# KLab/YAIK

Measured on AMD Instinct MI355X. Metric: Mpix/s tile encode (alpha reject + 7 gradient passes + 8x8 range quant), 8K RGBA, higher is better.
Workload: dtype u8/int32 (+f32 mode-selection sums)

## Files before the change

yaik_amd/csrc/yk_encode2.hip:

```cpp
#include "yk_common.h"
#include "yk_curves.h"
#include "yk_device.h"
#include <mutex>

__constant__ float c_curve2[6][16] = YK_CURVE_TABLE;

#define LS YK_LSTRIDE
#ifdef YK_TEST_HOOKS
#define YK2_ABLATE(bit) ((P.ablate & (bit)) != 0)
#else
#define YK2_ABLATE(bit) false
#endif

__device__ __forceinline__ int y2_byte(uint32_t w, int ch) { return (w >> (8 * ch)) & 255; }
__device__ __forceinline__ uint32_t y2_absdiff(uint32_t a, uint32_t b) { uint32_t r; asm("v_sad_u32 %0, %1, %2, 0" : "=v"(r) : "v"(a), "v"(b)); return r; }
__device__ __forceinline__ int y2_round6(int v) { return (v & ~3) | (v >> 6); }
__device__ __forceinline__ int y2_round6p(int v) { v = min(v + 1, 255); return (v & ~3) | (v >> 6); }

typedef short y2s2 __attribute__((ext_vector_type(2)));
typedef unsigned short y2u2 __attribute__((ext_vector_type(2)));
__device__ __forceinline__ y2u2 y2_u2(uint32_t w) { return __builtin_bit_cast(y2u2, w); }
__device__ __forceinline__ y2s2 y2_s2(y2u2 v) { return __builtin_bit_cast(y2s2, v); }
__device__ __forceinline__ y2u2 y2_splat(int v) { const unsigned short t = (unsigned short)v; return (y2u2){ t, t }; }
__device__ __forceinline__ y2s2 y2_splats(int v) { const short t = (short)v; return (y2s2){ t, t }; }
__device__ __forceinline__ y2s2 y2_rg(uint32_t p) { return y2_s2(y2_u2(__builtin_amdgcn_perm(0u, p, 0x010C000Cu) ^ 0x80008000u)); }
__device__ __forceinline__ y2s2 y2_bb(uint32_t pEven, uint32_t pOdd) { return y2_s2(y2_u2(__builtin_amdgcn_perm(pOdd, pEven, 0x060C020Cu) ^ 0x80008000u)); }
#define YK2_LATN 85
#ifdef YK2_STATS
__device__ unsigned long long g_y2_stats[192];
#define YK2_STAT(i, n) do { if (lane == 0) atomicAdd(&g_y2_stats[(i)], (unsigned long long)(n)); } while (0)
extern "C" int yk_debug_path_stats(unsigned long long* out, int clear) {
    hipError_t e = hipMemcpyFromSymbol(out, HIP_SYMBOL(g_y2_stats), sizeof(g_y2_stats));
    if (e == hipSuccess && clear) { static unsigned long long z[192]; e = hipMemcpyToSymbol(HIP_SYMBOL(g_y2_stats), z, sizeof(z)); }
    return (int)e;
}
#else
#define YK2_STAT(i, n) do { } while (0)
#endif

__device__ __forceinline__ constexpr int y2_cell_x(int m) { return (m & 1) | ((m >> 1) & 2); }
__device__ __forceinline__ constexpr int y2_cell_y(int m) { return ((m >> 1) & 1) | ((m >> 2) & 2); }
template <int NX, int NY> __device__ __forceinline__ constexpr unsigned long long y2_origin() {
    unsigned long long m = 0;
    for (int i = 0; i < 16; i++) if ((y2_cell_x(i) % NX) == 0 && (y2_cell_y(i) % NY) == 0) m |= 1ULL << i;
    return m * 0x0001000100010001ULL;
}
template <int NX, int NY> __device__ __forceinline__ unsigned long long y2_fold(unsigned long long m) {
    if (NX >= 2) m |= m >> 1;
    if (NY >= 2) m |= m >> 2;
    if (NX == 4) m |= m >> 4;
    if (NY == 4) m |= m >> 8;
    return m;
}
template <int NX, int NY> __device__ __forceinline__ unsigned long long y2_spread(unsigned long long m) {
    if (NX >= 2) m |= m << 1;
    if (NY >= 2) m |= m << 2;
    if (NX == 4) m |= m << 4;
    if (NY == 4) m |= m << 8;
    return m;
}

__device__ __forceinline__ constexpr int y2_pass_sx(int id) { return id < 2 ? 4 : (id < 5 ? 3 : 2); }
__device__ __forceinline__ constexpr int y2_pass_sy(int id) { return id == 0 || id == 2 ? 4 : (id == 1 || id == 3 || id == 5 ? 3 : 2); }
template <int SX, int SY> __device__ __forceinline__ constexpr int y2_pass_id() {
    for (int id = 0; id < 7; id++) if (y2_pass_sx(id) == SX && y2_pass_sy(id) == SY) return id;
    return -1;
}
struct Y2Pass {
    const uint32_t* s_lat; int lat;
    int cx, cy;
    const y2s2 (&rg)[16]; const y2s2 (&bb)[8];
    unsigned long long deadLanes; bool stripInside;
    int gxCell, gyCell, w, h;
    int rf;
    uint32_t* s_bm; int bxCell, byCell;
    const uint32_t* s_pix; uint8_t* s_list; uint32_t* s_tf;
    int lane;
};
struct Y2Window { y2s2 loO, hiO, loR, hiR; };
__device__ __forceinline__ Y2Window y2_window(const int rf) {
    const int loO = -256 * rf, hiO = 256 * rf + 255;
    return { y2_splats(loO), y2_splats(hiO), y2_splats(loO - 127), y2_splats(hiO - 127) };
}
template <int SX, int SY> __device__ __forceinline__ unsigned long long y2_viable(const Y2Pass pass, const unsigned long long cov) {
    constexpr int TX = 1 << SX, TY = 1 << SY, NX = TX / 4, NY = TY / 4;
    unsigned long long viable = y2_origin<NX, NY>() & ~cov & ~y2_fold<NX, NY>(pass.deadLanes);
    if (!pass.stripInside) {
        const int tgx = pass.gxCell - (pass.cx & (NX - 1)) * 4, tgy = pass.gyCell - (pass.cy & (NY - 1)) * 4;
        viable &= __ballot((tgx + TX <= pass.w) && (tgy + TY <= pass.h));
    }
    return viable;
}
template <int SX, int SY> __device__ __forceinline__ int y2_bitmap_bit(const int bxCell, const int byCell) {
    const int tbx = bxCell >> SX, tby = byCell >> SY;
    if (SX == 4 && SY == 4) return 0 + tby * 4 + tbx;
    if (SX == 4 && SY == 3) return 32 + tby * 4 + tbx;
    if (SX == 3 && SY == 4) return 64 + tby * 8 + tbx;
    if (SX == 3 && SY == 3) return 96 + tby * 8 + tbx;
    if (SX == 3 && SY == 2) return 160 + (tby >> 3) * 64 + (tby & 7) * 8 + tbx;
    if (SX == 2 && SY == 3) return 288 + (tbx >> 3) * 64 + tby * 8 + (tbx & 7);
    return 416 + ((tby >> 3) * 2 + (tbx >> 3)) * 64 + (tby & 7) * 8 + (tbx & 7);
}

template <int SX, int SY, int SXB = SX, int SYB = SY>
__device__ __forceinline__ void y2_accept(const Y2Pass pass, unsigned long long& cov, const unsigned long long accept, const unsigned long long acceptB = 0ULL) {
    cov |= y2_spread<(1 << SX) / 4, (1 << SY) / 4>(accept) | y2_spread<(1 << SXB) / 4, (1 << SYB) / 4>(acceptB);
    if ((accept | acceptB) != 0ULL && __builtin_amdgcn_inverse_ballot_w64(accept | acceptB)) {
        int bit = y2_bitmap_bit<SX, SY>(pass.bxCell, pass.byCell);
        if ((SXB != SX || SYB != SY) && __builtin_amdgcn_inverse_ballot_w64(acceptB)) bit = y2_bitmap_bit<SXB, SYB>(pass.bxCell, pass.byCell);
        atomicOr(&pass.s_bm[bit >> 5], 1u << (bit & 31));
    }
    __builtin_amdgcn_wave_barrier();
}

template <int SX, int SY>
__device__ __forceinline__ bool y2_compact_sweep(const Y2Pass pass, const unsigned long long viable, unsigned long long& cov, unsigned long long& evaluated) {
    constexpr int NX = (1 << SX) / 4, NY = (1 << SY) / 4, kPassId = y2_pass_id<SX, SY>();
    const uint32_t* const s_lat = pass.s_lat; const uint32_t* const s_pix = pass.s_pix; uint8_t* const s_list = pass.s_list; uint32_t* const s_tf = pass.s_tf;
    const int lane = pass.lane;
    const Y2Window W = y2_window(pass.rf);
    const unsigned long long cells = y2_spread<NX, NY>(viable);
    const int nCells = __popcll(cells);
    if (nCells > 16) return false;
    YK2_STAT(kPassId * 10 + 1, 1); YK2_STAT(kPassId * 10 + 7, nCells);
    constexpr bool kHasNext = kPassId >= 3 && kPassId <= 5;
    constexpr int SXB = kHasNext ? y2_pass_sx(kPassId + 1) : SX, SYB = kHasNext ? y2_pass_sy(kPassId + 1) : SY;
    constexpr int NXB = (1 << SXB) / 4, NYB = (1 << SYB) / 4;
    unsigned long long viableB = 0ULL, cellsB = 0ULL;
    int nB = 0;
#ifndef YK2_NO_GROUP
    if (kHasNext) {
        viableB = y2_viable<SXB, SYB>(pass, cov);
        cellsB = y2_spread<NXB, NYB>(viableB);
        nB = __popcll(cellsB);
        if (nB == 0 || nCells + nB > 16) { viableB = 0ULL; cellsB = 0ULL; nB = 0; }
    }
#endif
    const int rank = (int)__builtin_amdgcn_mbcnt_hi((uint32_t)(cells >> 32), __builtin_amdgcn_mbcnt_lo((uint32_t)cells, 0u));
    const bool mine = __builtin_amdgcn_inverse_ballot_w64(cells);
    if (mine) s_list[rank] = (uint8_t)lane;
    if (kHasNext && nB != 0) {
        YK2_STAT(140 + kPassId - 3, 1); YK2_STAT(150 + kPassId - 3, nB);
        const int rankB = (int)__builtin_amdgcn_mbcnt_hi((uint32_t)(cellsB >> 32), __builtin_amdgcn_mbcnt_lo((uint32_t)cellsB, 0u));
        if (__builtin_amdgcn_inverse_ballot_w64(cellsB)) s_list[nCells + rankB] = (uint8_t)lane;
    }
    s_tf[lane] = 0u; s_tf[64 + lane] = 0u;
    __builtin_amdgcn_fence(__ATOMIC_RELEASE, "wavefront"); __builtin_amdgcn_wave_barrier(); __builtin_amdgcn_fence(__ATOMIC_ACQUIRE, "wavefront");
    const int j = lane & 15, r = lane >> 4;
    const bool act = j < nCells + nB;
    const bool isB = kHasNext && j >= nCells;
    const int c = (int)s_list[act ? j : 0];
    const int q2 = c >> 4, cy2 = y2_cell_y(c & 15), cx2 = y2_cell_x(c & 15);
    constexpr int kInTile = (NX > 1 ? 1 : 0) | (NY > 1 ? 2 : 0) | (NX > 2 ? 4 : 0) | (NY > 2 ? 8 : 0);
    constexpr int kInTileB = (NXB > 1 ? 1 : 0) | (NYB > 1 ? 2 : 0) | (NXB > 2 ? 4 : 0) | (NYB > 2 ? 8 : 0);
    const int nxL = isB ? NXB : NX, nyL = isB ? NYB : NY;
    const int shx = isB ? 4 - SXB : 4 - SX, shy = isB ? 4 - SYB : 4 - SY;
    const int dcx2 = cx2 & (nxL - 1), dcy2 = cy2 & (nyL - 1);
    const int orig = c & ~(isB ? kInTileB : kInTile);
    const int fsh = isB ? 3 : 0;
    const int lo2 = cy2 * 17 + q2 * 4 + cx2 - dcy2 * 17 - dcx2;
    const int oTR = nxL, oBL = nyL * 17;
    const y2u2 wyr = y2_splat(16 - ((dcy2 * 4 + r) << shy));
    const y2u2 lxc = y2_splat(16 - ((dcx2 * 4) << shx));
    const y2u2 shx2 = y2_splat(shx);
    const uint4 pr = *reinterpret_cast<const uint4*>(&s_pix[(cy2 * 4 + r) * LS + q2 * 16 + cx2 * 4]);
    const y2s2 rgc[4] = { y2_rg(pr.x), y2_rg(pr.y), y2_rg(pr.z), y2_rg(pr.w) }, bbc[2] = { y2_bb(pr.x, pr.y), y2_bb(pr.z, pr.w) };
    y2s2 mnc[5], mxc[5];
    auto rowC = [&](const unsigned mask) {
        y2u2 Sc[5], stc[5];
#pragma unroll
        for (int t = 0; t < 5; t++) {
            if (!((mask >> t) & 1u)) continue;
            const uint32_t* lt = s_lat + t * YK2_LATN + lo2;
            const y2u2 TL = y2_u2(lt[0]), TR = y2_u2(lt[oTR]), BL = y2_u2(lt[oBL]), BR = y2_u2(lt[oBL + oTR]);
            const y2u2 e16 = (BL - BR) << 4, g = TR - BR, f = TL - BL - g;
            const y2u2 c2 = (g << 4) + f * lxc;
            Sc[t] = ((BR << 8) + e16 * lxc + c2 * wyr) ^ y2_splat(0x8000);
            stc[t] = (e16 + f * wyr) << shx2;
        }
#pragma unroll
        for (int i = 0; i < 4; i++) {
            const y2s2 c01 = rgc[i], cb = bbc[i >> 1];
            const y2s2 cc[4] = { __builtin_shufflevector(c01, c01, 0, 0), __builtin_shufflevector(c01, c01, 1, 1),
                                 (i & 1) ? __builtin_shufflevector(cb, cb, 1, 1) : __builtin_shufflevector(cb, cb, 0, 0), c01 };
#pragma unroll
            for (int t = 0; t < 4; t++) {
                if (!((mask >> t) & 1u)) continue;
                const y2s2 D = __builtin_elementwise_sub_sat(y2_s2(Sc[t]), cc[t]);
                if (i == 0) { mnc[t] = D; mxc[t] = D; }
                else { mnc[t] = __builtin_elementwise_min(mnc[t], D); mxc[t] = __builtin_elementwise_max(mxc[t], D); }
                if (i < 3) Sc[t] = Sc[t] - stc[t];
            }
        }
        if (mask & 0x10u) {
            const y2s2 Da = __builtin_elementwise_sub_sat(y2_s2(Sc[4] - stc[4] * (y2u2){ 0, 1 }), bbc[0]);
            const y2s2 Db = __builtin_elementwise_sub_sat(y2_s2(Sc[4] - stc[4] * (y2u2){ 2, 3 }), bbc[1]);
            mnc[4] = __builtin_elementwise_min(Da, Db); mxc[4] = __builtin_elementwise_max(Da, Db);
        }
    };
    constexpr uint32_t kAllFail = 0xE000E000u;
    auto failBits = [&](const y2s2 mnA, const y2s2 mxA, const y2s2 mnP, const y2s2 mxP) -> uint32_t {
        const y2s2 zero = y2_splats(0);
        const y2s2 oA = __builtin_elementwise_sub_sat(zero, __builtin_elementwise_max(__builtin_elementwise_sub_sat(W.loO, mnA), __builtin_elementwise_sub_sat(mxA, W.hiO)));
        const y2s2 rA = __builtin_elementwise_sub_sat(zero, __builtin_elementwise_max(__builtin_elementwise_sub_sat(W.loR, mnA), __builtin_elementwise_sub_sat(mxA, W.hiR)));
        const y2s2 oP = __builtin_elementwise_sub_sat(zero, __builtin_elementwise_max(__builtin_elementwise_sub_sat(W.loO, mnP), __builtin_elementwise_sub_sat(mxP, W.hiO)));
        const y2s2 rP = __builtin_elementwise_sub_sat(zero, __builtin_elementwise_max(__builtin_elementwise_sub_sat(W.loR, mnP), __builtin_elementwise_sub_sat(mxP, W.hiR)));
        const uint32_t a = __builtin_bit_cast(uint32_t, oA), b = __builtin_bit_cast(uint32_t, rA), cO = __builtin_bit_cast(uint32_t, oP), cR = __builtin_bit_cast(uint32_t, rP);
        uint32_t m = (a & 0x80008000u) | ((b >> 1) & 0x40004000u);
        m |= (((cO << 16) | cO) >> 2) & 0x20000000u;
        m |= (((cR >> 16) | cR) >> 2) & 0x00002000u;
        return m;
    };
    constexpr uint32_t kAllFailB = kAllFail >> 3;
    rowC(0x09u);
    if (act) atomicOr(&s_tf[orig], failBits(mnc[0], mxc[0], mnc[3], mxc[3]) >> fsh);
    __builtin_amdgcn_fence(__ATOMIC_RELEASE, "wavefront"); __builtin_amdgcn_wave_barrier(); __builtin_amdgcn_fence(__ATOMIC_ACQUIRE, "wavefront");
    const uint32_t w1 = s_tf[lane];
    const unsigned long long alive = viable & __ballot((kHasNext ? (w1 & kAllFail) : w1) != kAllFail);
    unsigned long long aliveB = 0ULL;
    if (kHasNext && nB != 0) aliveB = viableB & __ballot((w1 & kAllFailB) != kAllFailB);
    if ((alive | aliveB) == 0ULL) { YK2_STAT(100 + kPassId, 1); if (nB != 0) { YK2_STAT(146 + kPassId - 3, 1); YK2_STAT(143 + kPassId - 3, 1); } evaluated = viableB; return true; }
    rowC(0x16u);
    {
        const y2s2 mnA = __builtin_elementwise_min(__builtin_elementwise_min(mnc[0], mnc[1]), mnc[2]), mxA = __builtin_elementwise_max(__builtin_elementwise_max(mxc[0], mxc[1]), mxc[2]);
        const y2s2 mnP = __builtin_elementwise_min(mnc[3], mnc[4]), mxP = __builtin_elementwise_max(mxc[3], mxc[4]);
        if (act) atomicOr(&s_tf[64 + orig], failBits(mnA, mxA, mnP, mxP) >> fsh);
    }
    __builtin_amdgcn_fence(__ATOMIC_RELEASE, "wavefront"); __builtin_amdgcn_wave_barrier(); __builtin_amdgcn_fence(__ATOMIC_ACQUIRE, "wavefront");
    const uint32_t w2 = s_tf[64 + lane];
    const unsigned long long acceptC = alive & __ballot((kHasNext ? (w2 & kAllFail) : w2) != kAllFail);
    if (acceptC != 0ULL) { YK2_STAT(110 + kPassId, 1); }
    unsigned long long acceptB = 0ULL;
    if (kHasNext && nB != 0) {
        const unsigned long long covC = cov | y2_spread<NX, NY>(acceptC);
        const unsigned long long stillB = aliveB & ~covC;
        if (viableB & ~covC) YK2_STAT(143 + kPassId - 3, 1);
        acceptB = stillB & __ballot((w2 & kAllFailB) != kAllFailB);
        if (acceptB != 0ULL) { YK2_STAT(153 + kPassId - 3, 1); }
    }
    y2_accept<SX, SY, SXB, SYB>(pass, cov, acceptC, acceptB);
    evaluated = viableB;
    return true;
}

template <int SX, int SY, bool SMOOTH>
__device__ __forceinline__ unsigned long long y2_full_pass(const Y2Pass pass, unsigned long long viable) {
    constexpr int NX = (1 << SX) / 4, NY = (1 << SY) / 4, kPassId = y2_pass_id<SX, SY>();
    const uint32_t* const s_lat = pass.s_lat; const y2s2 (&rg)[16] = pass.rg; const y2s2 (&bb)[8] = pass.bb;
    const int lat = pass.lat, lane = pass.lane;
    const int dcx = pass.cx & (NX - 1), dcy = pass.cy & (NY - 1);
    const Y2Window W = y2_window(pass.rf);

    const int lo = lat - dcy * 17 - dcx;
    const y2u2 wy2 = y2_splat(16 - ((dcy * 4) << (4 - SY)));
    const y2u2 lx2 = y2_splat(16 - ((dcx * 4) << (4 - SX)));
    y2u2 S[4], st[4], dS0[4], dS3[4], dst[4], Sa, Sb, rsA, rsB;
    auto setup = [&](const int t) {
        const uint32_t* lt = s_lat + t * YK2_LATN + lo;
        const y2u2 TL = y2_u2(lt[0]), TR = y2_u2(lt[NX]), BL = y2_u2(lt[NY * 17]), BR = y2_u2(lt[NY * 17 + NX]);
        const y2u2 e16 = (BL - BR) << 4, g = TR - BR, f = TL - BL - g;
        const y2u2 c2 = (g << 4) + f * lx2;
        const y2u2 s0 = ((BR << 8) + e16 * lx2 + c2 * wy2) ^ y2_splat(0x8000);
        const y2u2 d0 = c2 << (4 - SY);
        const y2u2 sx = (e16 + f * wy2) << (4 - SX);
        const y2u2 dx = f << (8 - SX - SY);
        if (t < 4) {
            S[t] = s0; dS0[t] = d0; st[t] = sx; dst[t] = dx;
            dS3[t] = d0 - dx * (unsigned short)3;
        } else {
            const y2u2 k01 = { 0, 1 }, k23 = { 2, 3 };
            Sa = s0 - sx * k01; Sb = s0 - sx * k23;
            rsA = d0 - dx * k01; rsB = d0 - dx * k23;
        }
    };
    y2s2 mn[5], mx[5];
    auto pixelRow = [&](const int r, const unsigned mask, const bool first) {
        if (mask & 0x0Fu) {
#pragma unroll
            for (int ii = 0; ii < 4; ii++) {
                const int i = (r & 1) ? 3 - ii : ii;
                const y2s2 c01 = rg[r * 4 + i], cb = bb[r * 2 + (i >> 1)];
                const y2s2 cc[4] = { __builtin_shufflevector(c01, c01, 0, 0), __builtin_shufflevector(c01, c01, 1, 1),
                                     (i & 1) ? __builtin_shufflevector(cb, cb, 1, 1) : __builtin_shufflevector(cb, cb, 0, 0), c01 };
#pragma unroll
                for (int t = 0; t < 4; t++) {
                    if (!((mask >> t) & 1u)) continue;
                    const y2s2 D = __builtin_elementwise_sub_sat(y2_s2(S[t]), cc[t]);
                    if (first && ii == 0) { mn[t] = D; mx[t] = D; }
                    else { mn[t] = __builtin_elementwise_min(mn[t], D); mx[t] = __builtin_elementwise_max(mx[t], D); }
                    if (ii < 3) S[t] = (r & 1) ? S[t] + st[t] : S[t] - st[t];
                }
            }
        }
        if (mask & 0x10u) {
            const y2s2 Da = __builtin_elementwise_sub_sat(y2_s2(Sa), bb[r * 2]), Db = __builtin_elementwise_sub_sat(y2_s2(Sb), bb[r * 2 + 1]);
            const y2s2 lo4 = __builtin_elementwise_min(Da, Db), hi4 = __builtin_elementwise_max(Da, Db);
            if (first) { mn[4] = lo4; mx[4] = hi4; }
            else { mn[4] = __builtin_elementwise_min(mn[4], lo4); mx[4] = __builtin_elementwise_max(mx[4], hi4); }
        }
    };
    auto nextRow = [&](const int r, const unsigned mask) {
#pragma unroll
        for (int t = 0; t < 4; t++) if ((mask >> t) & 1u) { S[t] -= (r & 1) ? dS0[t] : dS3[t]; st[t] -= dst[t]; }
        if (mask & 0x10u) { Sa -= rsA; Sb -= rsB; }
    };
    auto failA4 = [&](const y2s2 mnA, const y2s2 mxA) -> unsigned long long {
        const y2s2 oA = __builtin_elementwise_max(__builtin_elementwise_sub_sat(W.loO, mnA), __builtin_elementwise_sub_sat(mxA, W.hiO));
        const y2s2 rA = __builtin_elementwise_max(__builtin_elementwise_sub_sat(W.loR, mnA), __builtin_elementwise_sub_sat(mxA, W.hiR));
        unsigned long long f = y2_fold<NX, NY>(__ballot(oA.x > 0));
        f &= y2_fold<NX, NY>(__ballot(oA.y > 0));
        f &= y2_fold<NX, NY>(__ballot(rA.x > 0));
        f &= y2_fold<NX, NY>(__ballot(rA.y > 0));
        return f;
    };
    auto failP2 = [&](const y2s2 mnP, const y2s2 mxP) -> unsigned long long {
        const y2s2 oP = __builtin_elementwise_max(__builtin_elementwise_sub_sat(W.loO, mnP), __builtin_elementwise_sub_sat(mxP, W.hiO));
        const y2s2 rP = __builtin_elementwise_max(__builtin_elementwise_sub_sat(W.loR, mnP), __builtin_elementwise_sub_sat(mxP, W.hiR));
        return y2_fold<NX, NY>(__ballot((oP.x > 0) | (oP.y > 0))) & y2_fold<NX, NY>(__ballot((rP.x > 0) | (rP.y > 0)));
    };
    auto mnAll = [&]() { return __builtin_elementwise_min(__builtin_elementwise_min(mn[0], mn[1]), mn[2]); };
    auto mxAll = [&]() { return __builtin_elementwise_max(__builtin_elementwise_max(mx[0], mx[1]), mx[2]); };

    constexpr bool kScreen = (NX * NY >= 4);
    constexpr unsigned kA = 0x07u, kP = 0x18u;
    unsigned long long accept;
    if (SMOOTH) {
        setup(0); setup(1); setup(2);
        pixelRow(0, kA, true);
        nextRow(0, kA); pixelRow(1, kA, false);
        nextRow(1, kA); pixelRow(2, kA, false);
        nextRow(2, kA); pixelRow(3, kA, false);
        YK2_STAT(kPassId * 10 + 4, 1);
        accept = viable & ~failA4(mnAll(), mxAll());
        const unsigned long long rest = viable & ~accept;
        if (rest != 0ULL) {
            YK2_STAT(kPassId * 10 + 5, 1); YK2_STAT(90 + kPassId, __popcll(y2_spread<NX, NY>(rest)));
            setup(3);
            pixelRow(0, 0x08u, true);
            const unsigned long long left = rest & ~failP2(mn[3], mx[3]);
            if (left != 0ULL) {
                setup(4);
                pixelRow(0, 0x10u, true);
                nextRow(0, kP); pixelRow(1, kP, false);
                nextRow(1, kP); pixelRow(2, kP, false);
                nextRow(2, kP); pixelRow(3, kP, false);
                accept |= left & ~failP2(__builtin_elementwise_min(mn[3], mn[4]), __builtin_elementwise_max(mx[3], mx[4]));
            }
        }
    } else {
        if (kScreen) {
            setup(0); setup(3);
            pixelRow(0, 0x09u, true);
            viable &= ~(failA4(mn[0], mx[0]) & failP2(mn[3], mx[3]));
            if (viable == 0ULL) { YK2_STAT(kPassId * 10 + 2, 1); return 0ULL; }
            setup(1); setup(2);
            pixelRow(0, 0x06u, true);
            viable &= ~(failA4(mnAll(), mxAll()) & failP2(mn[3], mx[3]));
            if (viable == 0ULL) { YK2_STAT(kPassId * 10 + 3, 1); return 0ULL; }
            nextRow(0, kA);
            pixelRow(1, kA, false);
        } else {
#pragma unroll
            for (int t = 0; t < 5; t++) setup(t);
            pixelRow(0, 0x1Fu, true);
            viable &= ~(failA4(mnAll(), mxAll()) & failP2(__builtin_elementwise_min(mn[3], mn[4]), __builtin_elementwise_max(mx[3], mx[4])));
            if (viable == 0ULL) { YK2_STAT(kPassId * 10 + 3, 1); return 0ULL; }
            nextRow(0, 0x1Fu);
            pixelRow(1, 0x1Fu, false);
            if (NX * NY <= 2) {
                viable &= ~(failA4(mnAll(), mxAll()) & failP2(__builtin_elementwise_min(mn[3], mn[4]), __builtin_elementwise_max(mx[3], mx[4])));
                if (viable == 0ULL) { YK2_STAT(kPassId * 10 + 9, 1); return 0ULL; }
            }
        }
        YK2_STAT(kPassId * 10 + 4, 1);
        nextRow(1, kA);
        pixelRow(2, kA, false);
        nextRow(2, kA);
        pixelRow(3, kA, false);
        accept = viable & ~failA4(mnAll(), mxAll());
        const unsigned long long rest = viable & ~accept;
        if (rest != 0ULL) {
            YK2_STAT(kPassId * 10 + 5, 1); YK2_STAT(90 + kPassId, __popcll(y2_spread<NX, NY>(rest)));
            if (kScreen) {
                setup(4);
                pixelRow(0, 0x10u, true);
                nextRow(0, kP);
                pixelRow(1, kP, false);
            }
            nextRow(1, kP);
            pixelRow(2, kP, false);
            nextRow(2, kP);
            pixelRow(3, kP, false);
            accept |= rest & ~failP2(__builtin_elementwise_min(mn[3], mn[4]), __builtin_elementwise_max(mx[3], mx[4]));
        }
    }
    return accept;
}

template <int SX, int SY, bool SMOOTH = false>
__device__ __forceinline__ void y2_grad_pass(const Y2Pass pass, unsigned long long& cov, unsigned long long& evaluated) {
    constexpr int NX = (1 << SX) / 4, NY = (1 << SY) / 4, kPassId = y2_pass_id<SX, SY>();
    const int lane = pass.lane;
    const unsigned long long viable = y2_viable<SX, SY>(pass, cov) & ~evaluated;
    evaluated = 0ULL;
    if (viable == 0ULL) return;
    YK2_STAT(kPassId * 10 + 0, 1); YK2_STAT(kPassId * 10 + 8, __popcll(y2_spread<NX, NY>(viable)));
    if (y2_compact_sweep<SX, SY>(pass, viable, cov, evaluated)) return;
    const unsigned long long accept = y2_full_pass<SX, SY, SMOOTH>(pass, viable);
    if (accept == 0ULL) return;
    YK2_STAT(kPassId * 10 + 6, 1);
    y2_accept<SX, SY>(pass, cov, accept);
}

#define YK2_QROWS 258
#define YK2_QR0 32
#define YK2_QNR 224
#define YK2_QBYTES ((size_t)YK2_QNR * YK2_QROWS * 16)
#define YK2_RCPBYTES ((size_t)256 * sizeof(float))
#define YK2_DEFN1 224
#define YK2_DEFBYTES ((size_t)225 * YK2_DEFN1 * 4)
#define YK2_TABBYTES (YK2_QBYTES + YK2_RCPBYTES + YK2_DEFBYTES)
typedef _Float16 y2h2 __attribute__((ext_vector_type(2)));
__device__ __forceinline__ uint32_t y2_f16_bits(int n) { const _Float16 h = (_Float16)(float)n; return (uint32_t)__builtin_bit_cast(unsigned short, h); }
__global__ void yk_qtab_kernel(uint4* tab) {
    __shared__ int K[6][16];
    const int R = YK2_QR0 + (int)blockIdx.x, t = threadIdx.x;
    if (t < 96) { const int m = t >> 4, i = t & 15; K[m][i] = __float2int_rz(__fmul_rn(c_curve2[m][i], (float)R)); }
    __syncthreads();
    if (t < YK2_QROWS) {
        const int o = t - 2;
        uint32_t md[6], idx = 0;
        for (int m = 0; m < 6; m++) {
            const int cnt = m < 3 ? 16 : 8;
            int best = 1 << 30, bi = 0;
            for (int n = 0; n < cnt; n++) { const int d = abs(K[m][n] - o); if (d < best) { best = d; bi = n; } }
            best = min(best, 255);
            md[m] = y2_f16_bits(best);
            idx |= (uint32_t)bi << (4 * m);
        }
        tab[(size_t)blockIdx.x * YK2_QROWS + t] = make_uint4(md[0] | (md[1] << 16), md[2] | (md[3] << 16), md[4] | (md[5] << 16), idx);
    }
}
struct Y2TileDef { int base, BN, dist, R; };
__device__ __forceinline__ Y2TileDef y2_tile_def(const int min_, const int d8) {
    Y2TileDef d;
    d.base = (min_ * 63 + 112) / 224;
    d.BN = (d.base * 224) / 63;
    const int scale = 223 - d.BN;
    const int dnum = (d8 - 32) * 127 + (scale - 1);
    d.dist = (scale < 0) ? -dnum : dnum / scale;
    d.R = (d.dist * scale) / 127 + 32;
    return d;
}
__global__ void yk_deftab_kernel(uint32_t* tab) {
    const int min_ = blockIdx.x, d8 = 32 + (int)threadIdx.x;
    const Y2TileDef d = y2_tile_def(min_, d8);
    const int R = min(max(d.R, YK2_QR0), YK2_QR0 + YK2_QNR - 1);
    const uint32_t rowBase = (uint32_t)((R - YK2_QR0) * YK2_QROWS + 2 - d.BN + 256);
    tab[min_ * YK2_DEFN1 + (int)threadIdx.x] = rowBase | (((((uint32_t)d.dist & 255u) << 7) | ((uint32_t)d.base & 255u)) << 16);
}

__global__ void yk_selftest_qtab_kernel(const uint4* tab, const uint32_t* deftab, int* mismatches) {
    const int mn = blockIdx.x, mx = threadIdx.x;
    if (mx < mn) return;
    const int min_ = min(mn, 224);
    int diff = mx - min_; if (diff < 16) diff = 16;
    const int d8 = max(diff, 32);
    const Y2TileDef d = y2_tile_def(min_, d8);
    const int BN = d.BN, R = d.R;
    int bad = 0;
    if (R < YK2_QR0 || R >= YK2_QR0 + YK2_QNR || mn - BN < -2) { atomicAdd(mismatches, 1); return; }
    {
        const uint32_t e = deftab[min_ * YK2_DEFN1 + (d8 - 32)];
        if ((e & 0xFFFFu) != (uint32_t)((R - YK2_QR0) * YK2_QROWS + 2 - BN + 256)) bad++;
        if ((e >> 16) != ((((uint32_t)d.dist & 255u) << 7) | ((uint32_t)d.base & 255u))) bad++;
    }
    for (int m = 0; m < 6; m++) {
        const int cnt = m < 3 ? 16 : 8;
        int L[16];
        for (int i = 0; i < cnt; i++) {
            L[i] = __float2int_rz(__fadd_rn((float)BN, __fmul_rn(c_curve2[m][i], (float)R)));
            if (L[i] != BN + __float2int_rz(__fmul_rn(c_curve2[m][i], (float)R))) bad++;
        }
        for (int v = mn; v <= mx; v++) {
            int best = 1 << 30, bi = 0;
            for (int n = 0; n < cnt; n++) { const int dd = abs(L[n] - v); if (dd < best) { best = dd; bi = n; } }
            const uint4 row = tab[(size_t)(R - YK2_QR0) * YK2_QROWS + (v - BN + 2)];
// ... 133 lines not shown
        const char* const b2 = reinterpret_cast<const char*>(pl2 + rowBase);
        int4 R[4], G[4], B[4];
#pragma unroll
        for (int k = 0; k < 4; k++) {
            const int rel = min(gyS + r0 + 4 * k, P.hAvail - 1) - gyB;
            const uint32_t off = (uint32_t)(rel * P.strideElems + gxc) * 4u;
            R[k] = *reinterpret_cast<const int4*>(b0 + off);
            G[k] = *reinterpret_cast<const int4*>(b1 + off);
            B[k] = *reinterpret_cast<const int4*>(b2 + off);
        }
        int4 Rb, Gb, Bb;
        {
            const int rel = min(gyS + 16, P.hAvail - 1) - gyB;
            const uint32_t off = (uint32_t)(rel * P.strideElems + gxc) * 4u;
            Rb = *reinterpret_cast<const int4*>(b0 + off);
            Gb = *reinterpret_cast<const int4*>(b1 + off);
            Bb = *reinterpret_cast<const int4*>(b2 + off);
        }
        uint32_t hcol;
        const int hr = min(max(lane - 32, 0), 16);
        {
            const int rel = min(gyS + hr, P.hAvail - 1) - gyB;
            const uint32_t off = (uint32_t)(rel * P.strideElems + min(BX * 64 + 64, w - 1)) * 4u;
            hcol = y2_pack3(*reinterpret_cast<const int32_t*>(b0 + off), *reinterpret_cast<const int32_t*>(b1 + off), *reinterpret_cast<const int32_t*>(b2 + off));
        }
        const float4 rc4 = *reinterpret_cast<const float4*>(P.qtab + YK2_QBYTES + (size_t)lane * 16);
        const uint4* const orow = P.outTab + (wave * YK2_OT_ROWS + (lane & (YK2_OT_ROWS - 1))) * 2;
        const uint4 ta = orow[0], tb = orow[1];
        {
            const bool rowIn = BY * 64 + wave * 16 < h;
            const uintptr_t args = reinterpret_cast<uintptr_t>(Pp);
            const uintptr_t kpIn = reinterpret_cast<uintptr_t>(P.keep) + fr * P.fs.keep + (uintptr_t)(mt0 & ~3);
            const uintptr_t bpIn = reinterpret_cast<uintptr_t>(P.bounds) + fr * 64;
            const uintptr_t kp = (P.keep != nullptr && rowIn) ? kpIn : args, bp = P.bounds != nullptr ? bpIn : args;
            asm volatile("s_load_dwordx2 %0, %2, 0x0\n\ts_load_dwordx4 %1, %3, 0x0" : "=&s"(keep8), "=&s"(bnd) : "s"(kp), "s"(bp));
        }

        __builtin_amdgcn_s_setprio(0);
        if (spare) return;
        {
            const uint32_t frT = frU + P.outFrame0;
            const uint32_t o = ta.x + frT * ta.y + (uint32_t)BX * ta.z + (uint32_t)BY * ta.w;
            s_park[lane] = ((uint32_t)BX < tb.x && (uint32_t)BY < tb.y) ? o : YK2_OT_NONE;
            s_park[64 + lane] = tb.z;
        }
        uint4 o[4], ob;
#pragma unroll
        for (int k = 0; k < 4; k++) {
            o[k] = make_uint4(y2_pack3(R[k].x, G[k].x, B[k].x), y2_pack3(R[k].y, G[k].y, B[k].y), y2_pack3(R[k].z, G[k].z, B[k].z), y2_pack3(R[k].w, G[k].w, B[k].w));
            *reinterpret_cast<uint4*>(&s_pix[(r0 + 4 * k) * LS + g4]) = o[k];
        }
        ob = make_uint4(y2_pack3(Rb.x, Gb.x, Bb.x), y2_pack3(Rb.y, Gb.y, Bb.y), y2_pack3(Rb.z, Gb.z, Bb.z), y2_pack3(Rb.w, Gb.w, Bb.w));
        if (lane < 16) *reinterpret_cast<uint4*>(&s_pix[16 * LS + g4]) = ob;
        if (BX * 64 + 64 > w) {
            if (!inX) {
#pragma unroll
                for (int k = 0; k < 4; k++) *reinterpret_cast<uint4*>(&s_pix[(r0 + 4 * k) * LS + g4]) = make_uint4(o[k].w, o[k].w, o[k].w, o[k].w);
                if (lane < 16) *reinterpret_cast<uint4*>(&s_pix[16 * LS + g4]) = make_uint4(ob.w, ob.w, ob.w, ob.w);
            }
        }
        if (lane >= 32 && lane <= 48) s_pix[hr * LS + 64] = hcol;
        *reinterpret_cast<float4*>(&s_rcp[lane * 4]) = rc4;

    }
    asm volatile("s_waitcnt lgkmcnt(0)" : "+s"(keep8), "+s"(bnd));
    __syncthreads();
    YK2_PROBE(1);

    const int q = lane >> 4, cx = y2_cell_x(lane & 15), cy = y2_cell_y(lane & 15);
    const int bxCell = q * 16 + cx * 4, byCell = wave * 16 + cy * 4;
    const int gxCell = BX * 64 + bxCell, gyCell = BY * 64 + byCell;
    const int lcell = (cy * 4) * LS + bxCell;
    const int lat = cy * 17 + q * 4 + cx;
    const bool mtIn = (BX * 64 + q * 16 < w) && (BY * 64 + wave * 16 < h);

    uint32_t pw[16];
#pragma unroll
    for (int r = 0; r < 4; r++) {
        const uint4 t = *reinterpret_cast<const uint4*>(&s_pix[lcell + r * LS]);
        pw[r * 4 + 0] = t.x; pw[r * 4 + 1] = t.y; pw[r * 4 + 2] = t.z; pw[r * 4 + 3] = t.w;
    }

    unsigned long long cov = 0ULL;
    unsigned long long evaluated = 0ULL;
    {
        bool dead = !mtIn;
        {
            const int lim = 4 * P.rejectFactor + 1;
            const y2u2 rb0 = y2_u2(pw[0] & 0x00FF00FFu), rb1 = y2_u2(pw[1] & 0x00FF00FFu), rb2 = y2_u2(pw[2] & 0x00FF00FFu), rb3 = y2_u2(pw[3] & 0x00FF00FFu);
            const y2u2 ga = y2_u2(__builtin_amdgcn_perm(pw[1], pw[0], 0x0C050C01u)), gb = y2_u2(__builtin_amdgcn_perm(pw[2], pw[1], 0x0C050C01u)),
                       gc = y2_u2(__builtin_amdgcn_perm(pw[3], pw[2], 0x0C050C01u));
            const y2u2 l2 = y2_splat(lim);
            const y2u2 u1 = rb0 + rb2 - rb1 - rb1 + l2, u2 = rb1 + rb3 - rb2 - rb2 + l2, ug = ga + gc - gb - gb + l2;
            const y2u2 um = __builtin_elementwise_max(__builtin_elementwise_max(u1, u2), ug);
            dead |= __builtin_bit_cast(uint32_t, __builtin_elementwise_sub_sat(um, y2_splat(2 * lim))) != 0u;
        }
        const unsigned long long deadLanes = __ballot(dead);
        YK2_STAT(75, 1); YK2_STAT(76, ~deadLanes == 0ULL ? 1 : 0); YK2_STAT(77, __popcll(deadLanes));
        const bool stripInside = (BX * 64 + 64 <= w) && (BY * 64 + wave * 16 + 16 <= h);
        if (~deadLanes != 0ULL && !YK2_ABLATE(2)) {
            auto latticePoint = [&](const int idx) {
                const int lr = (idx * 241) >> 12, lc = idx - lr * 17;
                const uint32_t raw = s_pix[(lr * 4) * LS + lc * 4];
                const uint32_t r6 = (raw & 0x00FCFCFCu) | ((raw >> 6) & 0x00030303u);
                const uint32_t z = (raw & 0x007F7F7Fu) + 0x00010101u;
                const uint32_t inc = (z ^ (raw & 0x00808080u)) | (((z & raw & 0x00808080u) >> 7) * 255u);
                const uint32_t p6 = (inc & 0x00FCFCFCu) | ((inc >> 6) & 0x00030303u);
                s_lat[0 * YK2_LATN + idx] = __builtin_amdgcn_perm(r6, raw, 0x0C040C00u);
                s_lat[1 * YK2_LATN + idx] = __builtin_amdgcn_perm(r6, raw, 0x0C050C01u);
                s_lat[2 * YK2_LATN + idx] = __builtin_amdgcn_perm(r6, raw, 0x0C060C02u);
                s_lat[3 * YK2_LATN + idx] = __builtin_amdgcn_perm(p6, p6, 0x0C010C00u);
                s_lat[4 * YK2_LATN + idx] = __builtin_amdgcn_perm(p6, p6, 0x0C020C02u);
            };
            latticePoint(lane);
            if (lane < YK2_LATN - 64) latticePoint(lane + 64);
            __syncthreads();
            y2s2 rg[16], bb[8];
#pragma unroll
            for (int k = 0; k < 16; k++) rg[k] = y2_rg(pw[k]);
#pragma unroll
            for (int k = 0; k < 8; k++) bb[k] = y2_bb(pw[2 * k], pw[2 * k + 1]);
            const Y2Pass S = { s_lat, lat, cx, cy, rg, bb, deadLanes, stripInside, gxCell, gyCell, w, h, P.rejectFactor, s_bm, bxCell, byCell, s_pix, s_list, s_range, lane };
            if (deadLanes == 0ULL) y2_grad_pass<4, 4, true>(S, cov, evaluated);
            else y2_grad_pass<4, 4>(S, cov, evaluated);
            if (~(cov | deadLanes) != 0ULL) {
                y2_grad_pass<4, 3>(S, cov, evaluated);
                y2_grad_pass<3, 4>(S, cov, evaluated);
                y2_grad_pass<3, 3>(S, cov, evaluated);
                y2_grad_pass<3, 2>(S, cov, evaluated);
                y2_grad_pass<2, 3>(S, cov, evaluated);
                y2_grad_pass<2, 2>(S, cov, evaluated);
            }
#pragma unroll
            for (int r = 0; r < 4; r++) {
                const uint4 t = *reinterpret_cast<const uint4*>(&s_pix[lcell + r * LS]);
                pw[r * 4 + 0] = t.x; pw[r * 4 + 1] = t.y; pw[r * 4 + 2] = t.z; pw[r * 4 + 3] = t.w;
            }
        }
    }
    const int mtIdx = mt0 + q;
    __syncthreads();
    YK2_PROBE(2);
    uint8_t* const small = P.small;
    const uint32_t tabOff = s_park[lane], tabSel = s_park[64 + lane];
    const uint32_t tabVal = (s_bm[tabSel & 31u] >> ((tabSel >> 8) & 31u)) & (~0u >> (tabSel >> 16));
    uint32_t off32 = (uint32_t)lane - 8u < 5u ? tabOff : ~0u;
    uint32_t val32 = (uint32_t)lane - 8u < 3u ? tabVal : 0u;
    {
        if ((uint32_t)lane - 1u < 3u) *(small + tabOff) = (uint8_t)tabVal;
        const unsigned long long t = ((cov >> 2) ^ cov) & 0x0C0C0C0C0C0C0C0CULL;
        const unsigned long long covRM = cov ^ t ^ (t << 2);
        uint32_t off16 = ((lane & 15) == 0 && mtIn) ? P.oCov + (frU * (uint32_t)P.fs.coverage + (uint32_t)mtIdx) * 2u : ~0u;
        uint32_t val16 = (uint32_t)((covRM >> (q * 16)) & 0xFFFFULL);
        if ((uint32_t)lane - 4u < 3u) { off16 = tabOff; val16 = tabVal; }
        if (off16 != ~0u) *reinterpret_cast<uint16_t*>(small + off16) = (uint16_t)val16;
        if (P.pixCache != nullptr) {
            const bool cellIn = (gxCell < w) && (gyCell < h);
            if (cellIn && !((cov >> lane) & 1ULL)) {
                const uint32_t strip = (uint32_t)((BY * 4 + wave) * P.xBB64 + BX);
                uint4* dstp = P.pixCache + (size_t)strip * 256 + lane;
#pragma unroll
                for (int r = 0; r < 4; r++) dstp[r * 64] = make_uint4(pw[r * 4 + 0], pw[r * 4 + 1], pw[r * 4 + 2], pw[r * 4 + 3]);
            }
        }
    }
    YK2_PROBE(3);
    int cxB = 0, cyB = 0, cw = w, chh = P.fullH, discard = 1;
    if (P.bounds != nullptr) {
        const int b0 = bnd.x, b1 = bnd.y, b2 = bnd.z, b3 = bnd.w;
        discard = (b0 == 0 && b1 == 0 && b2 == w && b3 == P.fullH) ? 1 : 0;
        cxB = (b0 >> 3) << 3; cyB = (b1 >> 3) << 3;
        cw = (((b2 + 7) >> 3) << 3) - cxB; chh = (((b3 + 7) >> 3) << 3) - cyB;
    }
    const int cxl = cx & 1, cyl = cy & 1;
    const int tgx = gxCell - cxl * 4, tgyl = gyCell - cyl * 4, tgy = tgyl + P.y0;
    const bool tileIn = (tgx + 8 <= w) && (tgyl + 8 <= h);
    const bool part = tileIn && tgx >= cxB && tgx < cxB + cw && tgy >= cyB && tgy < cyB + chh && (tgx + 8 <= cw) && (tgy + 8 <= chh);
    const uint32_t keep4 = (uint32_t)((((unsigned long long)keep8.y << 32) | keep8.x) >> (8 * (mt0 & 3)));
    const bool keepMT = (P.keep == nullptr) || discard || (mtIn && ((keep4 >> (8 * q)) & 0xFFu) != 0u);
    const bool tileLive = part && keepMT;
    const int l00 = lane & ~3;
    const uint32_t quadN = (uint32_t)((~cov) >> l00) & 15u;
    const int v00 = (int)(quadN & 1u), v01 = (int)((quadN >> 2) & 1u);
    const bool valid = tileLive && ((quadN >> (lane & 3)) & 1u);
    const int nTop = __popc(quadN & 3u), nBot = __popc(quadN >> 2);
    const int tileIdx = (tgyl >> 3) * P.tilesW + (tgx >> 3);
    const size_t T8 = (size_t)P.tilesW * P.tilesH;
    const int tw = lane >> 2;
    const bool writer = ((lane & 3) == 0) && tileIn;
    const unsigned long long validMask = __ballot(valid);
    const bool fullTiles = !WANT_DST && __ballot(tileLive && quadN != 15u && quadN != 0u) == 0ULL;

    {
        const int n16 = (tileLive && !YK2_ABLATE(1)) ? (nTop + nBot) : 0;
        if ((P.tilesW & 7) == 0) {
            if (validMask != 0ULL) {
#pragma unroll
                for (int r = 0; r < 2; r++) {
                    const bool mine = writer && ((cy >> 1) == r);
                    const unsigned long long b0 = __ballot(mine && (n16 & 1)), b1 = __ballot(mine && (n16 & 2)), b2 = __ballot(mine && (n16 & 4));
                    const unsigned long long bd = __ballot(mine && n16 > 0);
                    val32 = y2_writelane((uint32_t)(__popcll(b0) + 2 * __popcll(b1) + 4 * __popcll(b2)) | ((uint32_t)__popcll(bd) << 16), 11 + r, val32);
                }
            }
        } else if (writer && n16 > 0) {
// ... 403 lines not shown
```

Baseline: 243,800.

## Reuse compacted cell binding across consecutive gradient passes in compact sweep

Splits the compact sweep into a bind step (lane list build and per-lane pixel gather) and an eval step. When the next pass's viable cells match the current compacted cell set, it reuses the bound pixels to run that pass immediately: pass 1 is followed by 3x4, and pass 3 with its grouped pass 4 is followed by 2x3 with 2x2. The evaluated mask becomes a 3-deep queue so later passes skip the tiles already handled. This saves repeated list building, LDS gathers and y2_rg/y2_bb unpacking, at the cost of extra viability checks and more register pressure. It also adds stats counters under YK2_STATS.

New measurement: 242,800. Within noise of the previous version (-0.4%).

```diff
diff --git a/yaik_amd/csrc/yk_encode2.hip b/yaik_amd/csrc/yk_encode2.hip
--- a/yaik_amd/csrc/yk_encode2.hip
+++ b/yaik_amd/csrc/yk_encode2.hip
@@ -27,11 +27,11 @@
 __device__ __forceinline__ y2s2 y2_bb(uint32_t pEven, uint32_t pOdd) { return y2_s2(y2_u2(__builtin_amdgcn_perm(pOdd, pEven, 0x060C020Cu) ^ 0x80008000u)); }
 #define YK2_LATN 85
 #ifdef YK2_STATS
-__device__ unsigned long long g_y2_stats[192];
+__device__ unsigned long long g_y2_stats[256];
 #define YK2_STAT(i, n) do { if (lane == 0) atomicAdd(&g_y2_stats[(i)], (unsigned long long)(n)); } while (0)
 extern "C" int yk_debug_path_stats(unsigned long long* out, int clear) {
     hipError_t e = hipMemcpyFromSymbol(out, HIP_SYMBOL(g_y2_stats), sizeof(g_y2_stats));
-    if (e == hipSuccess && clear) { static unsigned long long z[192]; e = hipMemcpyToSymbol(HIP_SYMBOL(g_y2_stats), z, sizeof(z)); }
+    if (e == hipSuccess && clear) { static unsigned long long z[256]; e = hipMemcpyToSymbol(HIP_SYMBOL(g_y2_stats), z, sizeof(z)); }
     return (int)e;
 }
 #else
@@ -76,6 +76,9 @@
     uint32_t* s_bm; int bxCell, byCell;
     const uint32_t* s_pix; uint8_t* s_list; uint32_t* s_tf;
     int lane;
+#ifdef YK2_STATS
+    unsigned long long* s_prev;
+#endif
 };
 struct Y2Window { y2s2 loO, hiO, loR, hiR; };
 __device__ __forceinline__ Y2Window y2_window(const int rf) {
@@ -113,43 +116,49 @@
     __builtin_amdgcn_wave_barrier();
 }
 
+struct Y2Bound {
+    int c;
+    int r; bool act, second;
+    y2s2 rgc[4], bbc[2];
+};
+__device__ __forceinline__ Y2Bound y2_compact_bind(const Y2Pass pass, const unsigned long long cells, const int nCells, const unsigned long long cellsB, const int nB) {
+    uint8_t* const s_list = pass.s_list;
+    const int lane = pass.lane;
+    const int rank = (int)__builtin_amdgcn_mbcnt_hi((uint32_t)(cells >> 32), __builtin_amdgcn_mbcnt_lo((uint32_t)cells, 0u));
+    const bool mine = __builtin_amdgcn_inverse_ballot_w64(cells);
+    if (mine) s_list[rank] = (uint8_t)lane;
+    if (nB != 0) {
+        const int rankB = (int)__builtin_amdgcn_mbcnt_hi((uint32_t)(cellsB >> 32), __builtin_amdgcn_mbcnt_lo((uint32_t)cellsB, 0u));
+        if (__builtin_amdgcn_inverse_ballot_w64(cellsB)) s_list[nCells + rankB] = (uint8_t)lane;
+    }
+    __builtin_amdgcn_fence(__ATOMIC_RELEASE, "wavefront"); __builtin_amdgcn_wave_barrier(); __builtin_amdgcn_fence(__ATOMIC_ACQUIRE, "wavefront");
+    Y2Bound B;
+    const int j = lane & 15;
+    B.r = lane >> 4;
+    B.act = j < nCells + nB;
+    B.second = j >= nCells;
+    B.c = (int)s_list[B.act ? j : 0];
+    const int q2 = B.c >> 4, cy2 = y2_cell_y(B.c & 15), cx2 = y2_cell_x(B.c & 15);
+    const uint4 pr = *reinterpret_cast<const uint4*>(&pass.s_pix[(cy2 * 4 + B.r) * LS + q2 * 16 + cx2 * 4]);
+    B.rgc[0] = y2_rg(pr.x); B.rgc[1] = y2_rg(pr.y); B.rgc[2] = y2_rg(pr.z); B.rgc[3] = y2_rg(pr.w);
+    B.bbc[0] = y2_bb(pr.x, pr.y); B.bbc[1] = y2_bb(pr.z, pr.w);
+    return B;
+}
 template <int SX, int SY>
-__device__ __forceinline__ bool y2_compact_sweep(const Y2Pass pass, const unsigned long long viable, unsigned long long& cov, unsigned long long& evaluated) {
+__device__ __forceinline__ void y2_compact_eval(const Y2Pass pass, const Y2Bound& B, const unsigned long long viable, const unsigned long long viableB, const int nB,
+                                                unsigned long long& cov) {
     constexpr int NX = (1 << SX) / 4, NY = (1 << SY) / 4, kPassId = y2_pass_id<SX, SY>();
-    const uint32_t* const s_lat = pass.s_lat; const uint32_t* const s_pix = pass.s_pix; uint8_t* const s_list = pass.s_list; uint32_t* const s_tf = pass.s_tf;
+    const uint32_t* const s_lat = pass.s_lat; uint32_t* const s_tf = pass.s_tf;
     const int lane = pass.lane;
     const Y2Window W = y2_window(pass.rf);
-    const unsigned long long cells = y2_spread<NX, NY>(viable);
-    const int nCells = __popcll(cells);
-    if (nCells > 16) return false;
-    YK2_STAT(kPassId * 10 + 1, 1); YK2_STAT(kPassId * 10 + 7, nCells);
     constexpr bool kHasNext = kPassId >= 3 && kPassId <= 5;
     constexpr int SXB = kHasNext ? y2_pass_sx(kPassId + 1) : SX, SYB = kHasNext ? y2_pass_sy(kPassId + 1) : SY;
     constexpr int NXB = (1 << SXB) / 4, NYB = (1 << SYB) / 4;
-    unsigned long long viableB = 0ULL, cellsB = 0ULL;
-    int nB = 0;
-#ifndef YK2_NO_GROUP
-    if (kHasNext) {
-        viableB = y2_viable<SXB, SYB>(pass, cov);
-        cellsB = y2_spread<NXB, NYB>(viableB);
-        nB = __popcll(cellsB);
-        if (nB == 0 || nCells + nB > 16) { viableB = 0ULL; cellsB = 0ULL; nB = 0; }
-    }
-#endif
-    const int rank = (int)__builtin_amdgcn_mbcnt_hi((uint32_t)(cells >> 32), __builtin_amdgcn_mbcnt_lo((uint32_t)cells, 0u));
-    const bool mine = __builtin_amdgcn_inverse_ballot_w64(cells);
-    if (mine) s_list[rank] = (uint8_t)lane;
-    if (kHasNext && nB != 0) {
-        YK2_STAT(140 + kPassId - 3, 1); YK2_STAT(150 + kPassId - 3, nB);
-        const int rankB = (int)__builtin_amdgcn_mbcnt_hi((uint32_t)(cellsB >> 32), __builtin_amdgcn_mbcnt_lo((uint32_t)cellsB, 0u));
-        if (__builtin_amdgcn_inverse_ballot_w64(cellsB)) s_list[nCells + rankB] = (uint8_t)lane;
-    }
     s_tf[lane] = 0u; s_tf[64 + lane] = 0u;
     __builtin_amdgcn_fence(__ATOMIC_RELEASE, "wavefront"); __builtin_amdgcn_wave_barrier(); __builtin_amdgcn_fence(__ATOMIC_ACQUIRE, "wavefront");
-    const int j = lane & 15, r = lane >> 4;
-    const bool act = j < nCells + nB;
-    const bool isB = kHasNext && j >= nCells;
-    const int c = (int)s_list[act ? j : 0];
+    const int r = B.r, c = B.c;
+    const bool act = B.act;
+    const bool isB = kHasNext && B.second;
     const int q2 = c >> 4, cy2 = y2_cell_y(c & 15), cx2 = y2_cell_x(c & 15);
     constexpr int kInTile = (NX > 1 ? 1 : 0) | (NY > 1 ? 2 : 0) | (NX > 2 ? 4 : 0) | (NY > 2 ? 8 : 0);
     constexpr int kInTileB = (NXB > 1 ? 1 : 0) | (NYB > 1 ? 2 : 0) | (NXB > 2 ? 4 : 0) | (NYB > 2 ? 8 : 0);
@@ -163,8 +172,7 @@
     const y2u2 wyr = y2_splat(16 - ((dcy2 * 4 + r) << shy));
     const y2u2 lxc = y2_splat(16 - ((dcx2 * 4) << shx));
     const y2u2 shx2 = y2_splat(shx);
-    const uint4 pr = *reinterpret_cast<const uint4*>(&s_pix[(cy2 * 4 + r) * LS + q2 * 16 + cx2 * 4]);
-    const y2s2 rgc[4] = { y2_rg(pr.x), y2_rg(pr.y), y2_rg(pr.z), y2_rg(pr.w) }, bbc[2] = { y2_bb(pr.x, pr.y), y2_bb(pr.z, pr.w) };
+    const y2s2 (&rgc)[4] = B.rgc; const y2s2 (&bbc)[2] = B.bbc;
     y2s2 mnc[5], mxc[5];
     auto rowC = [&](const unsigned mask) {
         y2u2 Sc[5], stc[5];
@@ -219,7 +227,7 @@
     const unsigned long long alive = viable & __ballot((kHasNext ? (w1 & kAllFail) : w1) != kAllFail);
     unsigned long long aliveB = 0ULL;
     if (kHasNext && nB != 0) aliveB = viableB & __ballot((w1 & kAllFailB) != kAllFailB);
-    if ((alive | aliveB) == 0ULL) { YK2_STAT(100 + kPassId, 1); if (nB != 0) { YK2_STAT(146 + kPassId - 3, 1); YK2_STAT(143 + kPassId - 3, 1); } evaluated = viableB; return true; }
+    if ((alive | aliveB) == 0ULL) { YK2_STAT(100 + kPassId, 1); if (nB != 0) { YK2_STAT(146 + kPassId - 3, 1); YK2_STAT(143 + kPassId - 3, 1); } return; }
     rowC(0x16u);
     {
         const y2s2 mnA = __builtin_elementwise_min(__builtin_elementwise_min(mnc[0], mnc[1]), mnc[2]), mxA = __builtin_elementwise_max(__builtin_elementwise_max(mxc[0], mxc[1]), mxc[2]);
@@ -239,7 +247,58 @@
         if (acceptB != 0ULL) { YK2_STAT(153 + kPassId - 3, 1); }
     }
     y2_accept<SX, SY, SXB, SYB>(pass, cov, acceptC, acceptB);
-    evaluated = viableB;
+}
+template <int SX, int SY>
+__device__ __forceinline__ bool y2_compact_sweep(const Y2Pass pass, const unsigned long long viable, unsigned long long& cov, unsigned long long (&evaluated)[3]) {
+    constexpr int NX = (1 << SX) / 4, NY = (1 << SY) / 4, kPassId = y2_pass_id<SX, SY>();
+    const int lane = pass.lane;
+    const unsigned long long cells = y2_spread<NX, NY>(viable);
+    const int nCells = __popcll(cells);
+    if (nCells > 16) return false;
+    YK2_STAT(kPassId * 10 + 1, 1); YK2_STAT(kPassId * 10 + 7, nCells);
+    constexpr bool kHasNext = kPassId >= 3 && kPassId <= 5;
+    constexpr int SXB = kHasNext ? y2_pass_sx(kPassId + 1) : SX, SYB = kHasNext ? y2_pass_sy(kPassId + 1) : SY;
+    unsigned long long viableB = 0ULL, cellsB = 0ULL;
+    int nB = 0;
+#ifndef YK2_NO_GROUP
+    if (kHasNext) {
+        viableB = y2_viable<SXB, SYB>(pass, cov);
+        cellsB = y2_spread<(1 << SXB) / 4, (1 << SYB) / 4>(viableB);
+        nB = __popcll(cellsB);
+        if (nB == 0 || nCells + nB > 16) { viableB = 0ULL; cellsB = 0ULL; nB = 0; }
+    }
+#endif
+    if (kHasNext && nB != 0) { YK2_STAT(140 + kPassId - 3, 1); YK2_STAT(150 + kPassId - 3, nB); }
+#ifdef YK2_STATS
+    {
+        const unsigned long long prevC = pass.s_prev[0], prevB = pass.s_prev[1];
+        if (prevC == cells) { YK2_STAT(170 + kPassId, 1); if (prevB == 0ULL) { YK2_STAT(180 + kPassId, 1); if (nB == 0) YK2_STAT(190 + kPassId, 1); } }
+        __builtin_amdgcn_wave_barrier();
+        if (lane == 0) { pass.s_prev[0] = cells; pass.s_prev[1] = cellsB; }
+    }
+#endif
+    const Y2Bound B = y2_compact_bind(pass, cells, nCells, cellsB, nB);
+    y2_compact_eval<SX, SY>(pass, B, viable, viableB, nB, cov);
+    evaluated[0] = viableB;
+#ifndef YK2_NO_KEEP
+    if constexpr (kPassId == 1) {
+        const unsigned long long viable2 = y2_viable<3, 4>(pass, cov);
+        if (viable2 != 0ULL && y2_spread<2, 4>(viable2) == cells) {
+            YK2_STAT(200 + 2, 1); YK2_STAT(2 * 10 + 0, 1); YK2_STAT(2 * 10 + 8, nCells); YK2_STAT(2 * 10 + 1, 1); YK2_STAT(2 * 10 + 7, nCells);
+            y2_compact_eval<3, 4>(pass, B, viable2, 0ULL, 0, cov);
+            evaluated[0] = viable2;
+        }
+    }
+    if constexpr (kPassId == 3) if (nB != 0) {
+        const unsigned long long viable5 = y2_viable<2, 3>(pass, cov), viable6 = y2_viable<2, 2>(pass, cov);
+        if (viable5 != 0ULL && y2_spread<1, 2>(viable5) == cells && viable6 == cellsB) {
+            YK2_STAT(200 + 5, 1); YK2_STAT(5 * 10 + 0, 1); YK2_STAT(5 * 10 + 8, nCells); YK2_STAT(5 * 10 + 1, 1); YK2_STAT(5 * 10 + 7, nCells);
+            YK2_STAT(140 + 2, 1); YK2_STAT(150 + 2, nB);
+            y2_compact_eval<2, 3>(pass, B, viable5, viable6, nB, cov);
+            evaluated[1] = viable5; evaluated[2] = viable6;
+        }
+    }
+#endif
     return true;
 }
 
@@ -338,6 +397,7 @@
             setup(3);
             pixelRow(0, 0x08u, true);
             const unsigned long long left = rest & ~failP2(mn[3], mx[3]);
+            { const int nRest = __popcll(y2_spread<NX, NY>(rest)); YK2_STAT(160, 1); YK2_STAT(161, nRest <= 16 ? 1 : 0); YK2_STAT(162, left != 0ULL ? 1 : 0); YK2_STAT(163, (left != 0ULL && nRest <= 16) ? 1 : 0); YK2_STAT(164, __popcll(y2_spread<NX, NY>(left))); (void)nRest; }
             if (left != 0ULL) {
                 setup(4);
                 pixelRow(0, 0x10u, true);
@@ -398,11 +458,11 @@
 }
 
 template <int SX, int SY, bool SMOOTH = false>
-__device__ __forceinline__ void y2_grad_pass(const Y2Pass pass, unsigned long long& cov, unsigned long long& evaluated) {
+__device__ __forceinline__ void y2_grad_pass(const Y2Pass pass, unsigned long long& cov, unsigned long long (&evaluated)[3]) {
     constexpr int NX = (1 << SX) / 4, NY = (1 << SY) / 4, kPassId = y2_pass_id<SX, SY>();
     const int lane = pass.lane;
-    const unsigned long long viable = y2_viable<SX, SY>(pass, cov) & ~evaluated;
-    evaluated = 0ULL;
+    const unsigned long long viable = y2_viable<SX, SY>(pass, cov) & ~evaluated[0];
+    evaluated[0] = evaluated[1]; evaluated[1] = evaluated[2]; evaluated[2] = 0ULL;
     if (viable == 0ULL) return;
     YK2_STAT(kPassId * 10 + 0, 1); YK2_STAT(kPassId * 10 + 8, __popcll(y2_spread<NX, NY>(viable)));
     if (y2_compact_sweep<SX, SY>(pass, viable, cov, evaluated)) return;
@@ -702,7 +762,7 @@
     }
 
     unsigned long long cov = 0ULL;
-    unsigned long long evaluated = 0ULL;
+    unsigned long long evaluated[3] = { 0ULL, 0ULL, 0ULL };
     {
         bool dead = !mtIn;
         {
@@ -740,7 +800,13 @@
             for (int k = 0; k < 16; k++) rg[k] = y2_rg(pw[k]);
 #pragma unroll
             for (int k = 0; k < 8; k++) bb[k] = y2_bb(pw[2 * k], pw[2 * k + 1]);
+#ifdef YK2_STATS
+            __shared__ unsigned long long s_prevSweep[2];
+            if (lane == 0) { s_prevSweep[0] = 0ULL; s_prevSweep[1] = 0ULL; }
+            const Y2Pass S = { s_lat, lat, cx, cy, rg, bb, deadLanes, stripInside, gxCell, gyCell, w, h, P.rejectFactor, s_bm, bxCell, byCell, s_pix, s_list, s_range, lane, s_prevSweep };
+#else
             const Y2Pass S = { s_lat, lat, cx, cy, rg, bb, deadLanes, stripInside, gxCell, gyCell, w, h, P.rejectFactor, s_bm, bxCell, byCell, s_pix, s_list, s_range, lane };
+#endif
             if (deadLanes == 0ULL) y2_grad_pass<4, 4, true>(S, cov, evaluated);
             else y2_grad_pass<4, 4>(S, cov, evaluated);
             if (~(cov | deadLanes) != 0ULL) {
```
